# justinruggles/flake

Measured on AMD Instinct MI355X. Metric: Msamples/s encoded, 16-bit stereo 44.1k blocksize 4096 LPC-8, higher is better.
Workload: dtype int64/f64; 1 GPU; configs[1]: stereo 16-bit 44.1 kHz, blocksize 4096, LPC max order 8 (level-5 params, order method MAX, partition orders 0-5, stereo estimate), synthetic resonator PCM resident in HBM; frames_per_gpu=4096, batches=one resident batch, outputs=subframe info + packed Rice residual sections, parallelism=frame-sharded x1

## Files before the change

flake_amd/csrc/k1_autocorr.hip:

```cpp
#include "device_util.h"
#include "lpc_reg.h"

#ifdef FHIP_STAMPS
FHIP_DEFINE_STAMP_READER(fhip_debug_read_stamps_k1)
#define ACC_DECL(v_, n_) unsigned long long v_[n_] = {}
#define ACC_ADD(v_, i_, a_, b_) v_[i_] += (b_) - (a_)
#define ACC_PUT(slot_, val_)                                                           \
    do {                                                                               \
        if (blockIdx.x == 0 && (threadIdx.x & 63) == 0) g_fhip_stamps[slot_] = (long long)(val_); \
    } while (0)
#define STAMP_HWID() ACC_PUT(16 + (threadIdx.x >> 6), __builtin_amdgcn_s_getreg((31 << 11) | 4))
#else
#define ACC_DECL(v_, n_) do { } while (0)
#define ACC_ADD(v_, i_, a_, b_) do { } while (0)
#define ACC_PUT(slot_, val_) do { } while (0)
#define STAMP_HWID() do { } while (0)
#endif

namespace fhip {
namespace {

constexpr int AC_TILE = 128;
constexpr int AC_HALO = 32;
constexpr int AC_STRIDE = 170;
constexpr int AC_GMAX = 12;
constexpr int AC_PER_LANE = AC_TILE / WAVE;
constexpr int AC_CH = 8;
constexpr int AC_WAVES = 4;

__device__ __forceinline__ void wave_lds_fence()
{
    __builtin_amdgcn_fence(__ATOMIC_RELEASE, "wavefront");
    __builtin_amdgcn_wave_barrier();
    __builtin_amdgcn_fence(__ATOMIC_ACQUIRE, "wavefront");
}

__global__ __launch_bounds__(AC_WAVES * WAVE)
void k_autocorr(const int32_t *__restrict__ smp, double *__restrict__ autoc,
                int nsub, int n, int maxlag, int G, int nl2, double c, const int32_t *__restrict__ dev_sub)
{
    __shared__ double s_buf[AC_WAVES][AC_GMAX * AC_STRIDE];
    nsub = dev_count(dev_sub, nsub);

    const int lane = threadIdx.x & 63;
    const int wv = threadIdx.x >> 6;
    double *buf = s_buf[wv];
    const int s0 = (blockIdx.x * AC_WAVES + wv) * G;
    if (s0 >= nsub) return;
    const int half = n >> 1;
    const int ntiles = (n + AC_TILE - 1) / AC_TILE;

    const int32_t *rowp[AC_GMAX];
#pragma unroll
    for (int q = 0; q < AC_GMAX; q++) rowp[q] = smp + (size_t)min(s0 + q, nsub - 1) * n;
    int32_t cur[AC_GMAX][AC_PER_LANE];

    const int g = lane / nl2, j = lane - g * nl2;
    const int L0 = 2 * j, L1 = 2 * j + 1;
    const bool chain = (g < G) && (s0 + g < nsub) && (L0 <= maxlag);
    const double *rowa = buf + (chain ? g : 0) * AC_STRIDE + AC_HALO;
    const double *pb = rowa - (chain ? L0 : 0);
    double accE0 = 1.0, accO0 = 1.0, accE1 = 1.0, accO1 = 1.0;
    double b1 = 0.0;

    auto issue_loads = [&](int tb) {
#pragma unroll
        for (int q = 0; q < AC_GMAX; q++)
#pragma unroll
            for (int u = 0; u < AC_PER_LANE; u++)
                cur[q][u] = rowp[q][min(tb + u * WAVE + lane, n - 1)];
    };

    for (int idx = lane; idx < AC_GMAX * AC_HALO; idx += WAVE)
        buf[(idx >> 5) * AC_STRIDE + (idx & 31)] = 0.0;
    issue_loads(0);

    for (int t = 0; t < ntiles; t++) {
        const int tb = t * AC_TILE;
#pragma unroll
        for (int u = 0; u < AC_PER_LANE; u++) {
            const int p = tb + u * WAVE + lane;
            const int ii = (p < half) ? p : (n - 1 - p);
            const bool valid = (p < n) && (ii < half);
            const double tt = c - (double)ii;
            const double w = valid ? (1.0 - (tt * tt)) : 0.0;
#pragma unroll
            for (int q = 0; q < AC_GMAX; q++)
                buf[q * AC_STRIDE + AC_HALO + u * WAVE + lane] = (double)cur[q][u] * w;
        }
        issue_loads(tb + AC_TILE);
        wave_lds_fence();

        const int kend = min(AC_TILE, n - tb);
        if (t > 0 && kend == AC_TILE) {
            constexpr int NS = AC_TILE / AC_CH;
            double A[AC_CH], B[AC_CH], P[2 * AC_CH];
            double b1n;
            auto rd = [&](int st, double (&a)[AC_CH], double (&b)[AC_CH]) {
#pragma unroll
                for (int u = 0; u < AC_CH; u++) { a[u] = rowa[st * AC_CH + u]; b[u] = pb[st * AC_CH + u]; }
            };
            rd(0, A, B);
            {
                double pbv = b1;
#pragma unroll
                for (int u = 0; u < AC_CH; u++) { P[2 * u] = A[u] * B[u]; P[2 * u + 1] = A[u] * pbv; pbv = B[u]; }
                b1n = pbv;
            }
            rd(1, A, B);
#pragma unroll
            for (int cidx = 0; cidx < NS; cidx++) {
                double An[AC_CH], Bn[AC_CH], Pn[2 * AC_CH];
                if (cidx + 2 < NS) rd(cidx + 2, An, Bn);
                __builtin_amdgcn_sched_barrier(0);
                double pbv = b1n;
#pragma unroll
                for (int u = 0; u < AC_CH; u += 2) {
                    accE0 = accE0 + P[2 * u];
                    if (cidx + 1 < NS) Pn[2 * u] = A[u] * B[u];
                    accE1 = accE1 + P[2 * u + 1];
                    if (cidx + 1 < NS) Pn[2 * u + 1] = A[u] * pbv;
                    accO0 = accO0 + P[2 * u + 2];
                    if (cidx + 1 < NS) Pn[2 * u + 2] = A[u + 1] * B[u + 1];
                    accO1 = accO1 + P[2 * u + 3];
                    if (cidx + 1 < NS) Pn[2 * u + 3] = A[u + 1] * B[u];
                    pbv = B[u + 1];
                }
                __builtin_amdgcn_sched_barrier(0);
                if (cidx + 1 < NS) {
                    b1n = pbv;
#pragma unroll
                    for (int u = 0; u < 2 * AC_CH; u++) P[u] = Pn[u];
                }
                if (cidx + 2 < NS) {
#pragma unroll
                    for (int u = 0; u < AC_CH; u++) { A[u] = An[u]; B[u] = Bn[u]; }
                }
            }
            b1 = pb[AC_TILE - 1];
        } else {
            double accH0 = 1.0, accH1 = 1.0;
            for (int k = 0; k < kend; k++) {
                const int p = tb + k;
                const double a = rowa[k], b0 = pb[k];
                const double p0 = a * b0, p1 = a * b1;
                if (p <= maxlag) {
                    if (p >= L0) accH0 = accH0 + p0;
                    if (p >= L1) accH1 = accH1 + p1;
                    if (p == maxlag) {
                        if ((maxlag + 1) & 1) { accO0 = accH0; accO1 = accH1; }
                        else { accE0 = accH0; accE1 = accH1; }
                    }
                } else if (p & 1) {
                    accO0 = accO0 + p0;
                    accO1 = accO1 + p1;
                } else {
                    accE0 = accE0 + p0;
                    accE1 = accE1 + p1;
                }
                b1 = b0;
            }
        }
        wave_lds_fence();
        {
            double hv[(AC_GMAX * AC_HALO) / WAVE];
#pragma unroll
            for (int r = 0; r < (AC_GMAX * AC_HALO) / WAVE; r++) {
                const int idx = lane + r * WAVE;
                hv[r] = buf[(idx >> 5) * AC_STRIDE + AC_TILE + (idx & 31)];
            }
            wave_lds_fence();
#pragma unroll
            for (int r = 0; r < (AC_GMAX * AC_HALO) / WAVE; r++) {
                const int idx = lane + r * WAVE;
                buf[(idx >> 5) * AC_STRIDE + (idx & 31)] = hv[r];
            }
        }
    }
    if (chain) {
        double *dst = autoc + (size_t)(s0 + g) * FHIP_MAX_LAGS;
        dst[L0] = accE0 + accO0;
        if (L1 <= maxlag) dst[L1] = accE1 + accO1;
    }
}

__global__ __launch_bounds__(AC_WAVES * WAVE)
void k_autocorr_ragged(const int32_t *__restrict__ smp, double *__restrict__ autoc, int nsub, int nch, int row_n,
                       int maxlag, const int32_t *__restrict__ frame_n, const double *__restrict__ frame_c,
                       const int32_t *__restrict__ dev_sub)
{
    __shared__ double s_buf[AC_WAVES][AC_HALO + AC_TILE];
    const int lane = threadIdx.x & 63, wv = threadIdx.x >> 6;
    const int s = blockIdx.x * AC_WAVES + wv;
    nsub = dev_count(dev_sub, nsub);
    if (s >= nsub) return;
    double *buf = s_buf[wv];
    const int f = s / nch;
    const int n = __builtin_amdgcn_readfirstlane(frame_n[f]);
    double *dst = autoc + (size_t)s * FHIP_MAX_LAGS;
    if (n <= maxlag) {
        if (lane <= maxlag) dst[lane] = 2.0;
        return;
    }
    const double c = frame_c[f];
    const int32_t *row = smp + (size_t)s * row_n;
    const int half = n >> 1;
    const int lag = min(lane, maxlag);
    double acc1 = 1.0, acc2 = 1.0;
    if (lane < AC_HALO) buf[lane] = 0.0;
    for (int tb = 0; tb < n; tb += AC_TILE) {
#pragma unroll
        for (int u = 0; u < AC_PER_LANE; u++) {
            const int p = tb + u * WAVE + lane;
            const int ii = (p < half) ? p : (n - 1 - p);
            const bool valid = (p < n) && (ii < half);
            const double tt = c - (double)ii;
            const double w = valid ? (1.0 - (tt * tt)) : 0.0;
            buf[AC_HALO + u * WAVE + lane] = (double)row[min(p, n - 1)] * w;
        }
        wave_lds_fence();
        const int kend = min(AC_TILE, n - tb);
        for (int k = 0; k < kend; k++) {
            const int p = tb + k;
            const double prod = buf[AC_HALO + k] * buf[AC_HALO + k - lag];
            if (p <= maxlag) {
                if (p >= lag) acc1 = acc1 + prod;
            } else if ((p - maxlag) & 1) {
                acc1 = acc1 + prod;
            } else {
                acc2 = acc2 + prod;
            }
        }
        wave_lds_fence();
        const double hv = (lane < AC_HALO) ? buf[AC_TILE + lane] : 0.0;
        wave_lds_fence();
        if (lane < AC_HALO) buf[lane] = hv;
    }
    if (lane <= maxlag) dst[lane] = acc1 + acc2;
}

constexpr int PS_HALF = AC_TILE / 2;
constexpr int PS_HH = AC_HALO / 2;
constexpr int PS_ROW = PS_HH + PS_HALF;
constexpr int PS_STRIDE = 2 * PS_ROW + 10;
constexpr int PS_GMAX = 8;
constexpr int PS_CH = 8;

__global__ __launch_bounds__(AC_WAVES * WAVE)
void k_autocorr_ps(const int32_t *__restrict__ smp, double *__restrict__ autoc,
                   int nsub, int n, int maxlag, int G, int lps, int ge, double c,
                   const int32_t *__restrict__ dev_sub)
{
    __shared__ double s_buf[AC_WAVES][PS_GMAX * PS_STRIDE];
    nsub = dev_count(dev_sub, nsub);

    const int lane = threadIdx.x & 63;
    const int wv = threadIdx.x >> 6;
    double *buf = s_buf[wv];
    const int s0 = (blockIdx.x * AC_WAVES + wv) * G;
    if (s0 >= nsub) return;
    const int half = n >> 1;
    const int ntiles = (n + AC_TILE - 1) / AC_TILE;

    const int32_t *rowp[PS_GMAX];
#pragma unroll
    for (int q = 0; q < PS_GMAX; q++) rowp[q] = smp + (size_t)min(s0 + q, nsub - 1) * n;
    int32_t cur[PS_GMAX][AC_PER_LANE];

    const int g = lane / lps, ql = lane - g * lps;
    const int pi = ql & 1, grp = ql >> 1;
    const int l0 = (grp < ge) ? 6 * grp : 1 + 6 * (grp - ge);
    const bool chain = (g < G) && (s0 + g < nsub) && (l0 <= maxlag);
    const bool ok1 = l0 + 2 <= maxlag, ok2 = l0 + 4 <= maxlag;
    const int pib = pi ^ (l0 & 1);
    const int sft = (l0 + pib - pi) / 2;
    const double *rowA = buf + (chain ? g : 0) * PS_STRIDE + pi * PS_ROW + PS_HH;
    const double *rowB = buf + (chain ? g : 0) * PS_STRIDE + pib * PS_ROW + PS_HH - (chain ? sft : 0);
    const int pih = (maxlag + 1) & 1;
    double S0 = 1.0, S1 = 1.0, S2 = 1.0;
    double b1 = 0.0, b2 = 0.0;

    auto issue_loads = [&](int tb) {
#pragma unroll
        for (int q = 0; q < PS_GMAX; q++)
#pragma unroll
            for (int u = 0; u < AC_PER_LANE; u++)
                cur[q][u] = rowp[q][min(tb + u * WAVE + lane, n - 1)];
    };
    auto slot = [&](int q, int x) { return q * PS_STRIDE + (x & 1) * PS_ROW + PS_HH + (x >> 1); };

    for (int idx = lane; idx < PS_GMAX * 2 * PS_HH; idx += WAVE) {
        const int q = idx / (2 * PS_HH), r = idx - q * 2 * PS_HH;
        buf[q * PS_STRIDE + (r / PS_HH) * PS_ROW + (r % PS_HH)] = 0.0;
    }
    issue_loads(0);

    for (int t = 0; t < ntiles; t++) {
        const int tb = t * AC_TILE;
#pragma unroll
        for (int u = 0; u < AC_PER_LANE; u++) {
            const int x = u * WAVE + lane;
            const int p = tb + x;
            const int ii = (p < half) ? p : (n - 1 - p);
            const bool valid = (p < n) && (ii < half);
            const double tt = c - (double)ii;
            const double w = valid ? (1.0 - (tt * tt)) : 0.0;
#pragma unroll
            for (int q = 0; q < PS_GMAX; q++) buf[slot(q, x)] = (double)cur[q][u] * w;
        }
        issue_loads(tb + AC_TILE);
        wave_lds_fence();

        const int kend = min(AC_TILE, n - tb);
        if (t > 0 && kend == AC_TILE) {
            constexpr int NS = PS_HALF / PS_CH;
            double A[PS_CH], B[PS_CH];
#pragma unroll
            for (int u = 0; u < PS_CH; u++) { A[u] = rowA[u]; B[u] = rowB[u]; }
#pragma unroll
            for (int st = 0; st < NS; st++) {
                double An[PS_CH], Bn[PS_CH];
                if (st + 1 < NS) {
#pragma unroll
                    for (int u = 0; u < PS_CH; u++) {
                        An[u] = rowA[(st + 1) * PS_CH + u];
                        Bn[u] = rowB[(st + 1) * PS_CH + u];
                    }
                }
                __builtin_amdgcn_sched_barrier(0);
#pragma unroll
                for (int u = 0; u < PS_CH; u++) {
                    const double p0 = A[u] * B[u], p1 = A[u] * b1, p2 = A[u] * b2;
                    S0 = S0 + p0;
                    S1 = S1 + p1;
                    S2 = S2 + p2;
                    b2 = b1;
                    b1 = B[u];
                }
                __builtin_amdgcn_sched_barrier(0);
                if (st + 1 < NS) {
#pragma unroll
                    for (int u = 0; u < PS_CH; u++) { A[u] = An[u]; B[u] = Bn[u]; }
                }
            }
        } else {
            if (t == 0 && pi == pih) {
                const int hend = min(maxlag, kend - 1);
                for (int x = 0; x <= hend; x++) {
                    const double a = buf[slot(chain ? g : 0, x)];
                    if (x >= l0) {
                        const double p0 = a * buf[slot(chain ? g : 0, x - l0)];
                        S0 = S0 + p0;
                    }
                    if (ok1 && x >= l0 + 2) {
                        const double p1 = a * buf[slot(chain ? g : 0, x - l0 - 2)];
                        S1 = S1 + p1;
                    }
                    if (ok2 && x >= l0 + 4) {
                        const double p2 = a * buf[slot(chain ? g : 0, x - l0 - 4)];
                        S2 = S2 + p2;
                    }
                }
            }
            for (int st = 0; st < PS_HALF; st++) {
                const int x = 2 * st + pi;
                const int p = tb + x;
                if (x >= kend) break;
                const double a = rowA[st], b0 = rowB[st];
                if (p > maxlag) {
                    const double c1 = (x - l0 - 2 >= -AC_HALO) ? buf[slot(chain ? g : 0, x - l0 - 2 + AC_HALO) - PS_HH] : 0.0;
                    const double c2 = (x - l0 - 4 >= -AC_HALO) ? buf[slot(chain ? g : 0, x - l0 - 4 + AC_HALO) - PS_HH] : 0.0;
                    const double p0 = a * b0, p1 = a * c1, p2 = a * c2;
                    S0 = S0 + p0;
                    S1 = S1 + p1;
                    S2 = S2 + p2;
                }
                b2 = b1;
                b1 = b0;
            }
        }
        wave_lds_fence();
        {
            constexpr int NH = (PS_GMAX * 2 * PS_HH) / WAVE;
            double hv[NH];
#pragma unroll
            for (int r = 0; r < NH; r++) {
                const int idx = lane + r * WAVE;
                const int q = idx / (2 * PS_HH), rr = idx - q * 2 * PS_HH;
                hv[r] = buf[q * PS_STRIDE + (rr / PS_HH) * PS_ROW + PS_HALF + (rr % PS_HH)];
            }
            wave_lds_fence();
#pragma unroll
            for (int r = 0; r < NH; r++) {
                const int idx = lane + r * WAVE;
                const int q = idx / (2 * PS_HH), rr = idx - q * 2 * PS_HH;
                buf[q * PS_STRIDE + (rr / PS_HH) * PS_ROW + (rr % PS_HH)] = hv[r];
            }
        }
    }
    const double o0 = __shfl_xor(S0, 1, WAVE), o1 = __shfl_xor(S1, 1, WAVE), o2 = __shfl_xor(S2, 1, WAVE);
    if (chain && pi == 0) {
        double *dst = autoc + (size_t)(s0 + g) * FHIP_MAX_LAGS;
        dst[l0] = S0 + o0;
        if (ok1) dst[l0 + 2] = S1 + o1;
        if (ok2) dst[l0 + 4] = S2 + o2;
    }
}

template <int NCH, bool FUSED, int LPCMO>
constexpr wt_split wt_split_of() { return (NCH == 3 && !FUSED && LPCMO == 8) ? WT_SPLIT_O8 : WT_SPLIT_EVEN; }
constexpr int WT_ROW = PS_HH + PS_HALF + 2;
constexpr int WT_STRIDE = 2 * WT_ROW + 2;
static_assert(WT_ROW % 2 == 0 && WT_STRIDE % 4 == 2, "16-byte aligned arrays, odd slot stride");
constexpr int WT_BUF = WT_SUB * WT_STRIDE;
constexpr int WT_NBUF = 3;
#ifndef FHIP_WT_AHEAD
#define FHIP_WT_AHEAD 3
#endif
constexpr int WT_AHEAD = FHIP_WT_AHEAD;

template <int TL>
struct wt_geo {
    static_assert(TL == AC_TILE || TL == 2 * AC_TILE, "tile length");
    static constexpr int HALF = TL / 2;
    static constexpr int ROW = PS_HH + HALF + 2;
    static constexpr int STRIDE = 2 * ROW + 2;
    static constexpr int BUF = WT_SUB * STRIDE;
    static constexpr int NBUF = (TL == AC_TILE) ? WT_NBUF : 2;
    static constexpr int UNITS = TL / AC_TILE;
    static constexpr int AHEAD = (TL == AC_TILE) ? WT_AHEAD : 4;
    static constexpr int UT = AHEAD / UNITS;
    static_assert(ROW % 2 == 0 && STRIDE % 4 == 2, "16-byte aligned arrays, odd slot stride");
    static_assert(AHEAD % UNITS == 0 && (TL == AC_TILE || UT % NBUF == 0), "whole tiles per trip");
};
static_assert(wt_geo<AC_TILE>::ROW == WT_ROW && wt_geo<AC_TILE>::BUF == WT_BUF, "the 128 form's geometry");
constexpr int WTL_TILE = 2 * AC_TILE;

struct wt_groups { int l0[4]; int nch[4]; };

#ifdef FHIP_PROBE_NOB
constexpr bool wt_probe_nob = true;
#else
constexpr bool wt_probe_nob = false;
#endif
#ifdef FHIP_PROBE_NOPROD
constexpr bool wt_probe_noprod = true;
#else
constexpr bool wt_probe_noprod = false;
#endif
#ifdef FHIP_PROBE_NOWALK
constexpr bool wt_probe_nowalk = true;
#else
constexpr bool wt_probe_nowalk = false;
#endif
#ifdef FHIP_PROBE_NOHALO
constexpr bool wt_probe_nohalo = true;
#else
constexpr bool wt_probe_nohalo = false;
#endif
struct wt_lpc_args { int precision, omethod; int32_t *coefs, *shift, *opt_order, *fin; int32_t *tile_ctr; };
template <int MO>
__device__ __forceinline__ void lpc_reg_one(const double (&ac)[MO + 1], int s, int max_order, int precision,
                                            int omethod, int32_t *__restrict__ coefs,
                                            int32_t *__restrict__ shift, int32_t *__restrict__ opt_order,
                                            int32_t *__restrict__ fin);

template <int NCH, bool FUSED, int LPCMO, int TL>
__device__ __forceinline__
void wt_body(const int32_t *__restrict__ smp, double *__restrict__ autoc,
             int nsub, int n, int maxlag, wt_groups grp, double c,
             const int32_t *__restrict__ pcm, int32_t *__restrict__ smp_out,
             const fhip_subframe_info *__restrict__ info, wt_lpc_args lpc, int narrow_ok,
             const int32_t *__restrict__ dev_sub, const MultiBin &mb, wt_groups grp1, int lsplit)
{
    using GEO = wt_geo<TL>;
    constexpr int T_HALF = GEO::HALF, T_ROW = GEO::ROW, T_STRIDE = GEO::STRIDE, T_BUF = GEO::BUF;
    constexpr int T_NBUF = GEO::NBUF, T_UNITS = GEO::UNITS, T_AHEAD = GEO::AHEAD, T_UT = GEO::UT;
    constexpr bool LONG = TL != AC_TILE;
    extern __shared__ __attribute__((aligned(16))) double wt_lds[];
    double *acbuf = wt_lds + T_NBUF * T_BUF;

    const int lane = threadIdx.x & 63;
    const int wv = threadIdx.x >> 6;
    int blk = blockIdx.x;
    if (mb.nbins) {
        const int k = find_bin(mb, blk);
        blk -= mb.wg0[k];
        n = mb.n[k];
        c = mb.c[k];
        narrow_ok = mb.narrow[k];
        nsub = __builtin_amdgcn_readfirstlane(mb.cnt[mb.cnt_ix[k]]);
        const size_t u0 = (size_t)mb.unit0[k];
        smp += mb.smp_off[k];
        autoc += u0 * FHIP_MAX_LAGS;
        info += u0;
        lpc.coefs += u0 * FHIP_MAX_ORDER * FHIP_MAX_ORDER;
        lpc.shift += u0 * FHIP_MAX_ORDER;
        lpc.opt_order += u0;
        lpc.fin += u0 * FIN_STRIDE;
    } else {
        nsub = dev_count(dev_sub, nsub);
    }
    if (lsplit == 2) {
        if (blk & 1) grp = grp1;
        blk >>= 1;
    }
    const int sub0 = blk * WT_SUB;
    if (sub0 >= nsub) return;
    const int half = n >> 1;
    const int ntiles = n / TL;
    const int ntiles_pad = ((ntiles + T_UT - 1) / T_UT) * T_UT;
    STAMP_HWID();

    if (wv >= 4) {
        auto produce = [&](auto nrows_c, int q0, auto allnar_c) {
            constexpr int NR = decltype(nrows_c)::value;
            constexpr bool ALLNAR = decltype(allnar_c)::value;
            constexpr int NL = FUSED ? (NR + 1) / 2 : NR;
            auto uni64 = [](unsigned long long v) {
                return ((unsigned long long)(unsigned)__builtin_amdgcn_readfirstlane((int)(v >> 32)) << 32) |
                       (unsigned)__builtin_amdgcn_readfirstlane((int)v);
            };
            unsigned long long rowb[NL], outb[NR];
            int mode[NL], w0s[NL], w1s[NL];
            int nar[NL];
#pragma unroll
            for (int r = 0; r < NL; r++) {
                if (FUSED) {
                    const int sub = min(sub0 + q0 + 2 * r, nsub - 2);
                    rowb[r] = uni64((unsigned long long)(pcm + (size_t)sub * n));
                    outb[2 * r] = uni64((unsigned long long)(smp_out + (size_t)sub * n));
                    outb[2 * r + 1] = uni64((unsigned long long)(smp_out + (size_t)(sub + 1) * n));
                    mode[r] = __builtin_amdgcn_readfirstlane(info[sub].ch_mode);
                    w0s[r] = __builtin_amdgcn_readfirstlane(info[sub].wasted);
                    w1s[r] = __builtin_amdgcn_readfirstlane(info[sub + 1].wasted);
                } else {
                    const int sub = min(sub0 + q0 + r, nsub - 1);
                    rowb[r] = uni64((unsigned long long)(smp + (size_t)sub * n));
                    nar[r] = narrow_ok ? (__builtin_amdgcn_readfirstlane(info[sub].reserved) & 0xFF) : 0;
                }
            }
            typedef typename std::conditional<FUSED, int4, int2>::type ld_t;
            ld_t pre[T_AHEAD][NL];
            auto issue_loads = [&](ld_t (&dst)[NL], int tb, bool pinned = false) {
                const int p = min(tb + 2 * lane, n - 2);
#pragma unroll
                for (int r = 0; r < NL; r++) {
                    const int idx = FUSED ? 2 * p : ((ALLNAR || nar[r]) ? (p >> 1) : p);
                    typedef const int32_t __attribute__((address_space(1))) *g_i32;
                    typedef int ldv_t __attribute__((ext_vector_type(FUSED ? 4 : 2)));
                    typedef const ldv_t __attribute__((address_space(1))) *g_ld;
                    if constexpr (ALLNAR) {
                        dst[r].x = *((g_i32)rowb[r] + idx);
                    } else {
                        const ldv_t v = *(g_ld)((g_i32)rowb[r] + idx);
                        __builtin_memcpy(&dst[r], &v, sizeof(ld_t));
                    }
                    if (pinned) __builtin_amdgcn_sched_barrier(0);
                }
            };
#pragma unroll
            for (int a = 0; a < T_AHEAD; a++) issue_loads(pre[a], a * AC_TILE, true);
            if constexpr (!LONG) {
                for (int idx = lane; idx < NR * 2 * PS_HH; idx += WAVE) {
                    const int r = idx / (2 * PS_HH), k = idx - r * 2 * PS_HH;
                    wt_lds[(q0 + r) * T_STRIDE + (k / PS_HH) * T_ROW + (k % PS_HH)] = 0.0;
                }
            }
            double hl0[LONG ? NR : 1], hl1[LONG ? NR : 1];
#pragma unroll
            for (int r = 0; r < (LONG ? NR : 1); r++) { hl0[r] = 0.0; hl1[r] = 0.0; }
            auto weight = [&](int p) {
                const int ii = (p < half) ? p : (n - 1 - p);
                const bool valid = (p < n) && (ii < half);
                const double tt = c - (double)ii;
                return valid ? (1.0 - (tt * tt)) : 0.0;
            };
            int bi = 0;
            ACC_DECL(pacc, 3);
            for (int t0 = 0; t0 < ntiles_pad; t0 += T_UT) {
#pragma unroll
                for (int a = 0; a < T_UT; a++) {
                    const int bnx = (bi == T_NBUF - 1) ? 0 : bi + 1;
                    const bool tail = lane >= PS_HALF - PS_HH;
                    if (LONG && tail && !wt_probe_nohalo && !wt_probe_noprod) {
                        double *bh = wt_lds + bi * T_BUF + q0 * T_STRIDE + lane - (PS_HALF - PS_HH);
#pragma unroll
                        for (int r = 0; r < NR; r++) {
                            bh[r * T_STRIDE] = hl0[LONG ? r : 0];
                            bh[r * T_STRIDE + T_ROW] = hl1[LONG ? r : 0];
                        }
                    }
#pragma unroll
                    for (int h = 0; h < T_UNITS; h++) {
                        TICK(tp0);
                        const int ai = a * T_UNITS + h;
                        const int tb = (t0 + a) * TL + h * AC_TILE;
                        double *bw = wt_lds + bi * T_BUF + q0 * T_STRIDE + PS_HH + h * PS_HALF + lane;
                        double *bn = wt_lds + bnx * T_BUF + q0 * T_STRIDE + PS_HH + lane - PS_HALF;
                        const double w0 = weight(tb + 2 * lane), w1 = weight(tb + 2 * lane + 1);
                        const int pst = min(tb + 2 * lane, n - 2);
                        double hv0[NR], hv1[NR];
#pragma unroll
                        for (int r = 0; r < (wt_probe_noprod ? 0 : NR); r++) {
                            int32_t x0, x1;
                            if (FUSED) {
                                const int4 v = *reinterpret_cast<const int4 *>(&pre[ai][r / 2]);
                                const int md = mode[r / 2];
                                const int32_t s0 = (int32_t)((uint32_t)v.x - (uint32_t)v.y);
                                const int32_t s1 = (int32_t)((uint32_t)v.z - (uint32_t)v.w);
                                if ((r & 1) == 0) {
                                    const int32_t m0 = (int32_t)((uint32_t)v.x + (uint32_t)v.y) >> 1;
                                    const int32_t m1 = (int32_t)((uint32_t)v.z + (uint32_t)v.w) >> 1;
                                    x0 = (md == FHIP_CH_MID_SIDE) ? m0 : (md == FHIP_CH_RIGHT_SIDE) ? s0 : v.x;
                                    x1 = (md == FHIP_CH_MID_SIDE) ? m1 : (md == FHIP_CH_RIGHT_SIDE) ? s1 : v.z;
                                    x0 >>= w0s[r / 2]; x1 >>= w0s[r / 2];
                                } else {
                                    x0 = (md == FHIP_CH_MID_SIDE || md == FHIP_CH_LEFT_SIDE) ? s0 : v.y;
                                    x1 = (md == FHIP_CH_MID_SIDE || md == FHIP_CH_LEFT_SIDE) ? s1 : v.w;
                                    x0 >>= w1s[r / 2]; x1 >>= w1s[r / 2];
                                }
                                *reinterpret_cast<int2 *>(reinterpret_cast<int32_t *>(outb[r]) + pst) = make_int2(x0, x1);
                            } else {
                                const int2 v = *reinterpret_cast<const int2 *>(&pre[ai][r]);
                                const bool nr = ALLNAR || nar[FUSED ? 0 : r] != 0;
                                x0 = nr ? (int32_t)(int16_t)v.x : v.x;
                                x1 = nr ? (v.x >> 16) : v.y;
                            }
                            const double v0 = (double)x0 * w0;
                            const double v1 = (double)x1 * w1;
#ifdef FHIP_PROBE_NOLDSW
                            if (r == 0) { hv0[0] = 0; hv1[0] = 0; }
                            hv0[0] += v0; hv1[0] += v1;
                            if (r == NR - 1) { bw[0] = hv0[0]; bw[T_ROW] = hv1[0]; }
#else
                            bw[r * T_STRIDE] = v0;
                            bw[r * T_STRIDE + T_ROW] = v1;
                            hv0[r] = v0; hv1[r] = v1;
#endif
                        }
                        if constexpr (LONG) {
                            if (h == T_UNITS - 1) {
#pragma unroll
                                for (int r = 0; r < NR; r++) { hl0[r] = hv0[r]; hl1[r] = hv1[r]; }
                            }
                        } else if (tail && !wt_probe_nohalo && !wt_probe_noprod) {
#pragma unroll
                            for (int r = 0; r < NR; r++) {
                                bn[r * T_STRIDE] = hv0[r];
                                bn[r * T_STRIDE + T_ROW] = hv1[r];
                            }
                        }
                        TICK(tp1);
                        issue_loads(pre[ai], tb + T_AHEAD * AC_TILE);
                        TICK(tp2);
                        ACC_ADD(pacc, 0, tp0, tp1); ACC_ADD(pacc, 1, tp1, tp2);
                        if (h < T_UNITS - 1) {
                            __builtin_amdgcn_sched_barrier(0);
                        }
                    }
                    TICK(tp2);
                    __syncthreads();
                    TICK(tp3);
                    ACC_ADD(pacc, 2, tp2, tp3);
                    __builtin_amdgcn_sched_barrier(0);
                    bi = bnx;
                }
            }
            ACC_PUT(wv - 4, pacc[0]); ACC_PUT(wv, pacc[1]); ACC_PUT(wv + 4, pacc[2]);
            if (wv == 4) { ACC_PUT(44, pacc[0]); ACC_PUT(45, pacc[1]); ACC_PUT(46, pacc[2]); }
        };
        constexpr wt_split SP = wt_split_of<NCH, FUSED, LPCMO>();
        static_assert(wt_split_valid(SP), "producer row split");
        const int q0w = (wv == 4) ? 0 : (wv == 5) ? wt_split_first(SP, 1) : (wv == 6) ? wt_split_first(SP, 2)
                                                                                      : wt_split_first(SP, 3);
        const int nrw = (wv == 4) ? SP.rows[0] : (wv == 5) ? SP.rows[1] : (wv == 6) ? SP.rows[2] : SP.rows[3];
        bool alln = !FUSED && narrow_ok != 0;
        if (alln) {
            const int wide = (info[min(sub0 + q0w + min(lane, nrw - 1), nsub - 1)].reserved & 0xFF) == 0;
            alln = __ballot(wide) == 0;
        }
        auto produce_rows = [&](auto kc) {
            constexpr int K = decltype(kc)::value;
            if constexpr (wt_split_first_with(SP, K)) {
                if (nrw == SP.rows[K]) {
                    if (alln) produce(std::integral_constant<int, SP.rows[K]>{}, q0w, std::true_type{});
                    else produce(std::integral_constant<int, SP.rows[K]>{}, q0w, std::false_type{});
                }
            }
        };
        produce_rows(std::integral_constant<int, 0>{});
        produce_rows(std::integral_constant<int, 1>{});
        produce_rows(std::integral_constant<int, 2>{});
        produce_rows(std::integral_constant<int, 3>{});
        if (LPCMO > 0) __syncthreads();
        return;
    }

    const int pi = lane >> 5, sl = lane & 31;
    const int l0 = wv == 0 ? grp.l0[0] : wv == 1 ? grp.l0[1] : wv == 2 ? grp.l0[2] : grp.l0[3];
    const int nch = wv == 0 ? grp.nch[0] : wv == 1 ? grp.nch[1] : wv == 2 ? grp.nch[2] : grp.nch[3];
    const bool live = (sub0 + sl < nsub) && nch > 0;
    const int pib = pi ^ (l0 & 1);
    const int sft = (l0 + pib - pi) / 2;
    const int offA = sl * T_STRIDE + pi * T_ROW + PS_HH;
    const int offB = sl * T_STRIDE + pib * T_ROW + PS_HH - sft;
    const int pih = (maxlag + 1) & 1;
    auto slotc = [&](int x) { return sl * T_STRIDE + (x & 1) * T_ROW + PS_HH + (x >> 1); };
    double S[NCH], cy[NCH];
#pragma unroll
    for (int j = 0; j < NCH; j++) { S[j] = 1.0; cy[j] = 0.0; }

    auto walk_tile = [&](const double *rowA_, const double *rowB_, auto first, auto same, auto histc, auto kc,
                         auto &hist) {
        constexpr bool FIRST = decltype(first)::value;
        constexpr bool SAME = decltype(same)::value;
        constexpr int HD = decltype(histc)::value;
        constexpr int K = decltype(kc)::value;
        constexpr bool NOB = SAME || HD > 0 || wt_probe_nob;
        constexpr int NS = T_HALF / PS_CH;
        constexpr int DEPTH = (K <= 3) ? 2 : 1;
        constexpr int NSET = DEPTH + 1;
        typedef const volatile double __attribute__((address_space(3))) lds_cvd;
        typedef double dbl2 __attribute__((ext_vector_type(2)));
        typedef const volatile dbl2 __attribute__((address_space(3))) lds_cvd2;
        lds_cvd2 *rowA = (lds_cvd2 *)rowA_;
        lds_cvd *rowB = (lds_cvd *)rowB_;
        double A[NSET][PS_CH], B[NSET][PS_CH];
        int maxlag_v = maxlag;
        if constexpr (FIRST) asm volatile("" : "+v"(maxlag_v));
        auto fetch = [&](int set, int stage) {
#pragma unroll
            for (int u = 0; u < PS_CH; u += 2) {
                const dbl2 v = rowA[(stage * PS_CH + u) / 2];
                A[set][u] = v.x; A[set][u + 1] = v.y;
            }
            if (!NOB) {
#pragma unroll
                for (int u = 0; u < PS_CH; u++) B[set][u] = rowB[stage * PS_CH + u];
            }
        };
        constexpr int PER_STAGE = PS_CH / 2 + (NOB ? 0 : PS_CH);
        auto stage = [&](int st, int set, bool ahead, int newer, bool headz) __attribute__((always_inline)) {
            if (ahead) fetch((set + DEPTH) % NSET, st + DEPTH);
            {
                constexpr int w1 = PER_STAGE > 15 ? 15 : PER_STAGE;
                constexpr int w2 = 2 * PER_STAGE > 15 ? 15 : 2 * PER_STAGE;
                constexpr int enc1 = (3 << 14) | (w1 << 8) | (7 << 4) | 0xF;
                constexpr int enc2 = (3 << 14) | (w2 << 8) | (7 << 4) | 0xF;
                constexpr int enc0 = (3 << 14) | (0 << 8) | (7 << 4) | 0xF;
                if (newer == 2) __builtin_amdgcn_s_waitcnt(enc2);
                else if (newer == 1) __builtin_amdgcn_s_waitcnt(enc1);
                else __builtin_amdgcn_s_waitcnt(enc0);
            }
            __builtin_amdgcn_sched_barrier(0);
#pragma unroll
            for (int u = 0; u < PS_CH; u++) {
                const double x = (SAME || wt_probe_nob) ? A[set][u] : (HD > 0) ? hist[HD > 0 ? HD - 1 : 0]
                                                                                : B[set][u];
                double a = A[set][u];
                if (FIRST && headz && 2 * (st * PS_CH + u) <= FHIP_MAX_ORDER)
                    a = (2 * (st * PS_CH + u) + pi > maxlag_v) ? a : 0.0;
                double pr[K];
                pr[0] = a * x;
#pragma unroll
                for (int j = 1; j < K; j++) pr[j] = a * cy[j];
#pragma unroll
                for (int j = 0; j < K; j++) S[j] = S[j] + pr[j];
#pragma unroll
                for (int j = K - 1; j >= 2; j--) cy[j] = cy[j - 1];
                if constexpr (K > 1) cy[1] = x;
                if constexpr (HD > 0) {
#pragma unroll
                    for (int k = HD - 1; k >= 1; k--) hist[k] = hist[k - 1];
                    hist[0] = A[set][u];
                }
            }
            __builtin_amdgcn_sched_barrier(0);
        };
        auto newer_of = [](int st) { return (st + DEPTH < NS ? 1 : 0) + ((DEPTH == 2 && st + 1 < NS) ? 1 : 0); };
#pragma unroll
        for (int k = 0; k < DEPTH; k++) fetch(k, k);
        if constexpr (!LONG) {
#pragma unroll
            for (int st = 0; st < NS; st++) stage(st, st % NSET, st + DEPTH < NS, newer_of(st), true);
        } else {
            constexpr int HEADST = FIRST ? ((FHIP_MAX_ORDER / 2 + PS_CH) / PS_CH + NSET - 1) / NSET * NSET : 0;
            constexpr int STEADY = (NS - DEPTH) / NSET * NSET;
            static_assert(HEADST <= STEADY && (!FIRST || HEADST * PS_CH * 2 > FHIP_MAX_ORDER), "head inside the peeled stages");
#pragma unroll
            for (int st = 0; st < HEADST; st++) stage(st, st % NSET, true, DEPTH, true);
#pragma unroll 1
            for (int st0 = HEADST; st0 < STEADY; st0 += NSET) {
#pragma unroll
                for (int s = 0; s < NSET; s++) stage(st0 + s, s, true, DEPTH, false);
            }
#pragma unroll
            for (int st = STEADY; st < NS; st++) stage(st, st % NSET, st + DEPTH < NS, newer_of(st), false);
        }
    };

    auto walk_all = [&](auto same, auto histc, auto kc) {
        constexpr int HD = decltype(histc)::value;
        double hist[HD > 0 ? HD : 1];
#pragma unroll
        for (int k = 0; k < (HD > 0 ? HD : 1); k++) hist[k] = 0.0;
        int bi = 0;
        ACC_DECL(cacc, 4);
        for (int t = 0; t < ntiles_pad; t++) {
            TICK(tc0);
            __syncthreads();
            TICK(tc1);
            ACC_ADD(cacc, 0, tc0, tc1);
            if (t == 0) ACC_ADD(cacc, 3, tc0, tc1);
            if (t >= ntiles || wt_probe_nowalk || nch <= 0) continue;
            const double *buf = wt_lds + bi * T_BUF;
            if (t == 0 && pi == pih) {
#ifndef FHIP_HEAD_LOOP
                if constexpr (LPCMO > 0 && NCH >= 3) {
                    double hd[LPCMO + 1], he[LPCMO + 1];
#pragma unroll
                    for (int x = 0; x <= LPCMO; x++) { hd[x] = buf[slotc(x)]; he[x] = buf[slotc(x - l0)]; }
#pragma unroll
                    for (int x = 0; x <= LPCMO; x++) {
                        const double a = (x <= maxlag) ? hd[x] : 0.0;
#pragma unroll
                        for (int j = 0; j < NCH; j++) {
                            if (x - 2 * j >= 0) {
                                const double pr = a * he[x - 2 * j];
                                S[j] = S[j] + pr;
                            }
                        }
                    }
                } else
#endif
                for (int x = 0; x <= maxlag; x++) {
                    const double a = buf[slotc(x)];
#pragma unroll
                    for (int j = 0; j < NCH; j++) {
                        const int lag = l0 + 2 * j;
                        if (j < nch && x >= lag) {
                            const double pr = a * buf[slotc(x - lag)];
                            S[j] = S[j] + pr;
                        }
                    }
                }
            }
            if (t == 0) walk_tile(buf + offA, buf + offB, std::true_type{}, same, histc, kc, hist);
            else walk_tile(buf + offA, buf + offB, std::false_type{}, same, histc, kc, hist);
            bi = (bi == T_NBUF - 1) ? 0 : bi + 1;
            TICK(tc2);
            if (t == 0) ACC_ADD(cacc, 2, tc1, tc2);
            else ACC_ADD(cacc, 1, tc1, tc2);
        }
        ACC_PUT(48 + wv, cacc[1]); ACC_PUT(52 + wv, cacc[2]); ACC_PUT(56 + wv, cacc[0]); ACC_PUT(60 + wv, cacc[3]);
        if (wv == 0) { ACC_PUT(40, cacc[0]); ACC_PUT(41, cacc[1]); ACC_PUT(42, cacc[2]); }
    };

    using KF = std::integral_constant<int, NCH>;
    using KL = std::integral_constant<int, (NCH > 1) ? NCH - 1 : 1>;
    using H0 = std::integral_constant<int, 0>;
    using HN = std::integral_constant<int, NCH>;
    if (l0 == 0) {
        walk_all(std::true_type{}, H0{}, KF{});
    } else if (l0 == 2 * NCH) {
        if (nch == NCH) walk_all(std::false_type{}, HN{}, KF{});
        else walk_all(std::false_type{}, HN{}, KL{});
    } else if (nch == NCH) {
        walk_all(std::false_type{}, H0{}, KF{});
    } else {
        walk_all(std::false_type{}, H0{}, KL{});
    }
#pragma unroll
    for (int j = 0; j < NCH; j++) {
        const double o = __shfl_xor(S[j], 32, WAVE);
        if (live && pi == 0 && j < nch) {
            const double v = S[j] + o;
            autoc[(size_t)(sub0 + sl) * FHIP_MAX_LAGS + l0 + 2 * j] = v;
            if (LPCMO > 0) acbuf[sl * FHIP_MAX_LAGS + l0 + 2 * j] = v;
        }
    }
    if constexpr (LPCMO > 0) {
        bool tail_here = true;
        if (lsplit == 2) {
            asm volatile("s_waitcnt vmcnt(0)" ::: "memory");
            __syncthreads();
            int last = 0;
            if (threadIdx.x == 0) {
                __builtin_amdgcn_fence(__ATOMIC_RELEASE, "agent");
                asm volatile("s_waitcnt vmcnt(0)" ::: "memory");
                const int ticket = __hip_atomic_fetch_add(&lpc.tile_ctr[blk], 1, __ATOMIC_RELAXED, __HIP_MEMORY_SCOPE_AGENT);
                last = ticket & 1;
                if (last) {
                    __builtin_amdgcn_fence(__ATOMIC_ACQUIRE, "agent");
                    asm volatile("s_waitcnt vmcnt(0)" ::: "memory");
                }
            }
            tail_here = wv == 0 && __builtin_amdgcn_readfirstlane(last) != 0;
        } else {
            __syncthreads();
        }
        if (tail_here && wv == 0 && lane < WT_SUB && sub0 + lane < nsub) {
            double ac[LPCMO + 1];
            if (lsplit == 2) {
                const double *row = autoc + (size_t)(sub0 + lane) * FHIP_MAX_LAGS;
#pragma unroll
                for (int i = 0; i <= LPCMO; i++) ac[i] = (i <= maxlag) ? row[i] : 0.0;
            } else {
#pragma unroll
                for (int i = 0; i <= LPCMO; i++) ac[i] = (i <= maxlag) ? acbuf[lane * FHIP_MAX_LAGS + i] : 0.0;
            }
            lpc_reg_one<LPCMO>(ac, sub0 + lane, maxlag, lpc.precision, lpc.omethod, lpc.coefs, lpc.shift,
                               lpc.opt_order, lpc.fin);
        }
    }
}

#define WT_KERNEL_ARGS                                                                              \
    const int32_t *__restrict__ smp, double *__restrict__ autoc, int nsub, int n, int maxlag,       \
    wt_groups grp, double c, const int32_t *__restrict__ pcm, int32_t *__restrict__ smp_out,        \
    const fhip_subframe_info *__restrict__ info, wt_lpc_args lpc, int narrow_ok,                    \
    const int32_t *__restrict__ dev_sub, MultiBin mb, wt_groups grp1, int lsplit
#define WT_KERNEL_PASS smp, autoc, nsub, n, maxlag, grp, c, pcm, smp_out, info, lpc, narrow_ok, dev_sub, mb, grp1, lsplit

template <int NCH, bool FUSED, int LPCMO>
__global__ __launch_bounds__(8 * WAVE)
void k_autocorr_wt(WT_KERNEL_ARGS)
{
    wt_body<NCH, FUSED, LPCMO, AC_TILE>(WT_KERNEL_PASS);
}

template <int NCH, bool FUSED, int LPCMO>
__global__ __launch_bounds__(8 * WAVE)
void k_autocorr_wtl(WT_KERNEL_ARGS)
{
    wt_body<NCH, FUSED, LPCMO, WTL_TILE>(WT_KERNEL_PASS);
}
#undef WT_KERNEL_ARGS
#undef WT_KERNEL_PASS

}

namespace {
struct ac_choice { int kernel; int G, nl2, Gp, lps, ge, ne, no, split; };
ac_choice pick_autocorr(int nsub, int n, int max_order)
{
    ac_choice ch{};
    const int simds = 1024;
    ch.nl2 = (max_order + 2) / 2;
    ch.G = WAVE / ch.nl2;
    if (ch.G > AC_GMAX) ch.G = AC_GMAX;
    if (ch.G < 1) ch.G = 1;
    const long waves_cur = (nsub + ch.G - 1) / ch.G;
    ch.ne = max_order / 2 + 1; ch.no = (max_order + 1) / 2;
    ch.ge = (ch.ne + 2) / 3;
    const int go = (ch.no + 2) / 3;
    ch.lps = 2 * (ch.ge + go);
    ch.Gp = WAVE / ch.lps;
    if (ch.Gp > PS_GMAX) ch.Gp = PS_GMAX;
    const double t_cur = (double)((waves_cur + 2 * simds - 1) / (2 * simds)) *
                         (n * (waves_cur > simds ? 41.0 : 33.0) + 1000.0);
    const double t_ps = (ch.Gp >= 1) ? (double)(((nsub + ch.Gp - 1) / ch.Gp + simds - 1) / simds) * (0.5 * n * 39.0 + 1000.0) : 1e30;
    double t_wt = 1e30;
    ch.split = 1;
    if ((n % AC_TILE) == 0) {
        const int e0 = (ch.ne + 1) / 2;
        const double per_step = (4.8 * e0 > 23.0) ? 4.8 * e0 : 23.0;
        const int tiles = (nsub + WT_SUB - 1) / WT_SUB;
        t_wt = (double)((tiles + 255) / 256) * (0.5 * n * per_step + 8000.0);
        static const bool no_split = getenv("FHIP_NO_LAG_SPLIT") != nullptr;
        if (!no_split && 2 * tiles <= 256 && max_order >= 2) {
            ch.split = 2;
            const int m = (ch.ne + 3) / 4;
            const double ps2 = (4.8 * m > 14.0) ? 4.8 * m : 14.0;
            t_wt = 0.5 * n * ps2 + 8000.0;
        }
    }
    const double k2 = (max_order <= 12) ? 9000.0 : 0.0;
    ch.kernel = (t_wt <= t_ps + k2 && t_wt <= t_cur + k2) ? 2 : (t_ps < t_cur) ? 1 : 0;
    if (const char *force = getenv("FHIP_AC_KERNEL")) {
        if (force[0] == 'c') ch.kernel = 0;
        if (force[0] == 'p' && ch.Gp >= 1) ch.kernel = 1;
        if (force[0] == 'w' && (n % AC_TILE) == 0) ch.kernel = 2;
    }
    return ch;
}

bool wt_long_tile(const int *n, int count)
{
    const char *force = getenv("FHIP_WT_TILE");
    if (force && atoi(force) == AC_TILE) return false;
    for (int k = 0; k < count; k++) if (n[k] < WTL_TILE || (n[k] % WTL_TILE) != 0) return false;
    return true;
}
constexpr size_t wt_lds_bytes(bool long_tile)
{
    return sizeof(double) * (long_tile ? (size_t)wt_geo<WTL_TILE>::NBUF * wt_geo<WTL_TILE>::BUF
                                       : (size_t)WT_NBUF * WT_BUF);
}
static_assert(wt_lds_bytes(true) + sizeof(double) * WT_SUB * FHIP_MAX_LAGS <= 160 * 1024, "one workgroup's LDS");
}

}

extern "C" FHIP_API int fhip_autocorr_tile(int nsub, int n, int max_order)
{
    if (nsub < 1 || n < 1 || max_order < 1 || max_order > FHIP_MAX_ORDER) return 0;
    if (fhip::pick_autocorr(nsub, n, max_order).kernel != 2) return 0;
    return fhip::wt_long_tile(&n, 1) ? fhip::WTL_TILE : fhip::AC_TILE;
}

namespace fhip {

bool autocorr_is_wave_typed(int nsub, int n, int max_order)
{
    return pick_autocorr(nsub, n, max_order).kernel == 2;
}


bool autocorr_does_lpc(int nsub, int n, int max_order, bool have_tile_counters)
{
    static const bool off = getenv("FHIP_NO_LPC_TAIL") != nullptr;
    static const bool split_tail = getenv("FHIP_SPLIT_TAIL") != nullptr;
    if (off || max_order > 12) return false;
    const ac_choice ch = pick_autocorr(nsub, n, max_order);
    return ch.kernel == 2 && (ch.split == 1 || (have_tile_counters && split_tail));
}

bool autocorr_fuses_prepare(const fhip_params &p, int nsub, int n)
{
    static const bool on = getenv("FHIP_FUSE") != nullptr;
    if (!on || p.channels != 2 || (n & 3) != 0 || n > 4096 || (nsub & 1)) return false;
    return pick_autocorr(nsub, n, p.max_prediction_order).kernel == 2;
}

bool autocorr_bins_supported(int max_order, const int *n, int nbins)
{
    static const bool off = getenv("FHIP_NO_MULTIBIN") != nullptr;
    if (off || nbins < 1 || nbins > 8 || max_order < 1 || max_order > FHIP_MAX_ORDER) return false;
    for (int k = 0; k < nbins; k++) if (n[k] < AC_TILE || (n[k] % AC_TILE) != 0 || n[k] <= max_order) return false;
    return true;
}

hipError_t launch_autocorr_bins(hipStream_t st, const MultiBin &mb, const int32_t *smp, int max_order,
                                double *autoc, const fhip_subframe_info *info,
                                const autocorr_lpc_out *lpc_out)
{
    if (!autocorr_bins_supported(max_order, mb.n, mb.nbins)) return hipErrorInvalidValue;
    const int ne = max_order / 2 + 1, no = (max_order + 1) / 2;
    const int e0 = (ne + 1) / 2, e1 = ne - e0, o0 = (no + 1) / 2, o1 = no - o0;
    wt_groups gr;
    gr.l0[0] = 0;          gr.nch[0] = e0;
    gr.l0[1] = 2 * e0;     gr.nch[1] = e1;
    gr.l0[2] = 1;          gr.nch[2] = o0;
    gr.l0[3] = 1 + 2 * o0; gr.nch[3] = o1;
    const int nch = e0;
    const int blocks = mb.wg0[mb.nbins];
    if (blocks == 0) return hipSuccess;
    wt_lpc_args la{};
    int lpcmo = 0;
    if (lpc_out) {
        if (max_order > 12) return hipErrorInvalidValue;
        la.precision = lpc_out->precision; la.omethod = lpc_out->omethod;
        la.coefs = lpc_out->coefs; la.shift = lpc_out->shift; la.opt_order = lpc_out->opt_order;
        la.fin = lpc_out->fin;
        lpcmo = (max_order <= 8) ? 8 : 12;
    }
    const bool long_tile = wt_long_tile(mb.n, mb.nbins);
    const size_t lds = wt_lds_bytes(long_tile) + (lpcmo ? sizeof(double) * (size_t)WT_SUB * FHIP_MAX_LAGS : 0);
    bool any_narrow = false;
    for (int k = 0; k < mb.nbins; k++) any_narrow = any_narrow || mb.narrow[k];
#define LAUNCH_WTB(N_, L_)                                                                 \
    do {                                                                                     \
        auto kern = long_tile ? &k_autocorr_wtl<N_, false, L_> : &k_autocorr_wt<N_, false, L_>; \
        hipError_t er = hipFuncSetAttribute(reinterpret_cast<const void *>(kern),            \
                                            hipFuncAttributeMaxDynamicSharedMemorySize, (int)lds); \
        if (er != hipSuccess) return er;                                                     \
        note_launch("k_autocorr_wt<%d,false,%d> split=1%s%s", N_, L_, L_ ? " tail" : "", any_narrow ? " narrow" : ""); \
        hipLaunchKernelGGL(kern, dim3(blocks), dim3(8 * WAVE), lds, st, smp,                 \
                           autoc, 0, 0, max_order, gr, 0.0, (const int32_t *)nullptr, (int32_t *)nullptr, info, la, 0, \
                           (const int32_t *)nullptr, mb, wt_groups{}, 1);                    \
    } while (0)
    if (lpcmo == 8) {
        switch (nch) {
        case 1: LAUNCH_WTB(1, 8); break;
        case 2: LAUNCH_WTB(2, 8); break;
        case 3: LAUNCH_WTB(3, 8); break;
        default: return hipErrorInvalidValue;
        }
    } else if (lpcmo == 12) {
        switch (nch) {
        case 3: LAUNCH_WTB(3, 12); break;
        case 4: LAUNCH_WTB(4, 12); break;
        default: return hipErrorInvalidValue;
        }
    } else {
        switch (nch) {
        case 1: LAUNCH_WTB(1, 0); break;
        case 2: LAUNCH_WTB(2, 0); break;
        case 3: LAUNCH_WTB(3, 0); break;
        case 4: LAUNCH_WTB(4, 0); break;
        case 5: LAUNCH_WTB(5, 0); break;
        case 6: LAUNCH_WTB(6, 0); break;
        case 7: LAUNCH_WTB(7, 0); break;
        case 8: LAUNCH_WTB(8, 0); break;
        case 9: LAUNCH_WTB(9, 0); break;
        default: return hipErrorInvalidValue;
        }
    }
#undef LAUNCH_WTB
    return hipGetLastError();
}

hipError_t launch_autocorr_ragged(hipStream_t st, const int32_t *smp, int nsub, int nch, const RaggedFrames &rf,
                                  int max_order, double *autoc)
{
    if (nsub == 0) return hipSuccess;
    if (!rf.frame_n || !rf.frame_c || max_order < 1 || max_order > FHIP_MAX_ORDER) return hipErrorInvalidValue;
    note_launch("k_autocorr ragged");
    hipLaunchKernelGGL(k_autocorr_ragged, dim3((nsub + AC_WAVES - 1) / AC_WAVES), dim3(AC_WAVES * WAVE), 0, st, smp,
                       autoc, nsub, nch, rf.row_n, max_order, rf.frame_n, rf.frame_c, rf.dev_sub);
    return hipGetLastError();
}

hipError_t launch_autocorr(hipStream_t st, const int32_t *smp, int nsub, int n,
                           int max_order, double *autoc, const int32_t *pcm_fused,
                           int32_t *smp_out, const fhip_subframe_info *info,
                           const autocorr_lpc_out *lpc_out, bool narrow_ok, const int32_t *dev_sub,
                           int nsub_hint)
{
    if (nsub == 0) return hipSuccess;
    const double c = (2.0 / (n - 1.0)) - 1.0;
    const ac_choice ch = pick_autocorr(nsub_hint > 0 ? nsub_hint : nsub, n, max_order);
    const int ne = ch.ne, no = ch.no, Gp = ch.Gp, lps = ch.lps, ge = ch.ge, nl2 = ch.nl2;
    int G = ch.G;
    const bool use_wt = ch.kernel == 2, use_ps = ch.kernel == 1;
    if ((pcm_fused || lpc_out || narrow_ok) && !use_wt) return hipErrorInvalidValue;
    if (narrow_ok && (!info || pcm_fused)) return hipErrorInvalidValue;
    const int e0 = (ne + 1) / 2, e1 = ne - e0, o0 = (no + 1) / 2, o1 = no - o0;
    if (use_wt) {
        wt_groups gr, gr1{};
        const int split = (pcm_fused || (lpc_out && !lpc_out->tile_ctr)) ? 1 : ch.split;
        int nch;
        if (split == 2) {
            auto spread = [](wt_groups &g, int first, int count) {
                int l = first;
                for (int w = 0; w < 4; w++) {
                    const int k = count / 4 + (w < count % 4 ? 1 : 0);
                    g.l0[w] = l; g.nch[w] = k;
                    l += 2 * k;
                }
            };
            spread(gr, 0, ne);
            spread(gr1, 1, no);
            nch = (ne + 3) / 4;
        } else {
            gr.l0[0] = 0;          gr.nch[0] = e0;
            gr.l0[1] = 2 * e0;     gr.nch[1] = e1;
            gr.l0[2] = 1;          gr.nch[2] = o0;
            gr.l0[3] = 1 + 2 * o0; gr.nch[3] = o1;
            nch = e0;
        }
        const int blocks = split * ((nsub + WT_SUB - 1) / WT_SUB);
        const bool long_tile = !pcm_fused && wt_long_tile(&n, 1);
        const size_t lds = wt_lds_bytes(long_tile);
        wt_lpc_args la{};
        int lpcmo = 0;
        if (lpc_out) {
            if (max_order > 12 || pcm_fused) return hipErrorInvalidValue;
            la.precision = lpc_out->precision; la.omethod = lpc_out->omethod;
            la.coefs = lpc_out->coefs; la.shift = lpc_out->shift; la.opt_order = lpc_out->opt_order;
            la.fin = lpc_out->fin; la.tile_ctr = lpc_out->tile_ctr;
            lpcmo = (max_order <= 8) ? 8 : 12;
        }
        const size_t lds_all = lds + (lpcmo ? sizeof(double) * (size_t)WT_SUB * FHIP_MAX_LAGS : 0);
#define LAUNCH_WT3(N_, F_, L_)                                                               \
    do {                                                                                     \
        auto kern = (long_tile && !F_) ? &k_autocorr_wtl<N_, false, L_> : &k_autocorr_wt<N_, F_, L_>; \
        hipError_t er = hipFuncSetAttribute(reinterpret_cast<const void *>(kern),            \
                                            hipFuncAttributeMaxDynamicSharedMemorySize, (int)lds_all); \
        if (er != hipSuccess) return er;                                                     \
        note_launch("k_autocorr_wt<%d,%s,%d> split=%d%s%s%s", N_, tf(F_), L_, split, L_ ? " tail" : "", \
                    F_ ? " fused" : "", narrow_ok ? " narrow" : "");                         \
        hipLaunchKernelGGL(kern, dim3(blocks), dim3(8 * WAVE), lds_all, st, smp,             \
                           autoc, nsub, n, max_order, gr, c, pcm_fused, smp_out, info, la, narrow_ok ? 1 : 0, dev_sub, MultiBin{}, gr1, split); \
    } while (0)
#define LAUNCH_WT(N_)                                                                        \
    case N_:                                                                                 \
        if (pcm_fused) LAUNCH_WT3(N_, true, 0); else LAUNCH_WT3(N_, false, 0);               \
        break;
        if (lpcmo == 8) {
            switch (nch) {
            case 1: LAUNCH_WT3(1, false, 8); break;
            case 2: LAUNCH_WT3(2, false, 8); break;
            case 3: LAUNCH_WT3(3, false, 8); break;
            default: return hipErrorInvalidValue;
            }
            return hipGetLastError();
        }
        if (lpcmo == 12) {
            switch (nch) {
            case 2: LAUNCH_WT3(2, false, 12); break;
            case 3: LAUNCH_WT3(3, false, 12); break;
            case 4: LAUNCH_WT3(4, false, 12); break;
            default: return hipErrorInvalidValue;
            }
            return hipGetLastError();
        }
        switch (nch) {
            LAUNCH_WT(1) LAUNCH_WT(2) LAUNCH_WT(3) LAUNCH_WT(4) LAUNCH_WT(5)
            LAUNCH_WT(6) LAUNCH_WT(7) LAUNCH_WT(8) LAUNCH_WT(9)
        default: return hipErrorInvalidValue;
        }
#undef LAUNCH_WT
#undef LAUNCH_WT3
        return hipGetLastError();
    }
    if (use_ps) {
        const int per_block = Gp * AC_WAVES;
        const int blocks = (nsub + per_block - 1) / per_block;
        note_launch("k_autocorr_ps");
        hipLaunchKernelGGL(k_autocorr_ps, dim3(blocks), dim3(AC_WAVES * WAVE), 0, st, smp, autoc,
                           nsub, n, max_order, Gp, lps, ge, c, dev_sub);
        return hipGetLastError();
    }
    while (G > 1 && (nsub + G * AC_WAVES - 1) / (G * AC_WAVES) < 256) G--;
    if (const char *dbg = getenv("FHIP_AC_G")) { int v = atoi(dbg); if (v >= 1 && v <= AC_GMAX && v * nl2 <= WAVE) G = v; }
    const int per_block = G * AC_WAVES;
    const int blocks = (nsub + per_block - 1) / per_block;
    note_launch("k_autocorr");
    hipLaunchKernelGGL(k_autocorr, dim3(blocks), dim3(AC_WAVES * WAVE), 0, st, smp, autoc,
                       nsub, n, max_order, G, nl2, c, dev_sub);
    return hipGetLastError();
}

}
```

Before: 254,400 Msamples/s.

## Peel padded tail tiles, use byte offsets for loads, split LDS prefetch into early/late

The weighting loop is split so that full tiles run through a branch-free window weight, and only the final padded trip keeps the bounds checks. Global load addressing is rewritten to use precomputed unsigned byte offsets instead of per-row index arithmetic. In the autocorrelation stage pipeline, the A operands are kept as double2 vectors, and part of the next-stage LDS prefetch is deferred until the registers holding the tail data are free. The waitcnt thresholds are adjusted to match the new issue order. The aim is to cut ALU and addressing overhead and lower VGPR pressure, at the cost of more complex wait-count bookkeeping that could be gotten wrong.

```diff
diff --git a/flake_amd/csrc/k1_autocorr.hip b/flake_amd/csrc/k1_autocorr.hip
--- a/flake_amd/csrc/k1_autocorr.hip
+++ b/flake_amd/csrc/k1_autocorr.hip
@@ -544,16 +544,19 @@
             ld_t pre[T_AHEAD][NL];
             auto issue_loads = [&](ld_t (&dst)[NL], int tb, bool pinned = false) {
                 const int p = min(tb + 2 * lane, n - 2);
+                const unsigned off_w = (unsigned)p * (FUSED ? 8u : 4u);
+                const unsigned off_n = (unsigned)(p >> 1) * 4u;
 #pragma unroll
                 for (int r = 0; r < NL; r++) {
-                    const int idx = FUSED ? 2 * p : ((ALLNAR || nar[r]) ? (p >> 1) : p);
+                    const unsigned off = FUSED ? off_w : ((ALLNAR || nar[r]) ? off_n : off_w);
+                    typedef const char __attribute__((address_space(1))) *g_byte;
                     typedef const int32_t __attribute__((address_space(1))) *g_i32;
                     typedef int ldv_t __attribute__((ext_vector_type(FUSED ? 4 : 2)));
                     typedef const ldv_t __attribute__((address_space(1))) *g_ld;
                     if constexpr (ALLNAR) {
-                        dst[r].x = *((g_i32)rowb[r] + idx);
+                        dst[r].x = *(g_i32)((g_byte)rowb[r] + off);
                     } else {
-                        const ldv_t v = *(g_ld)((g_i32)rowb[r] + idx);
+                        const ldv_t v = *(g_ld)((g_byte)rowb[r] + off);
                         __builtin_memcpy(&dst[r], &v, sizeof(ld_t));
                     }
                     if (pinned) __builtin_amdgcn_sched_barrier(0);
@@ -570,15 +573,20 @@
             double hl0[LONG ? NR : 1], hl1[LONG ? NR : 1];
 #pragma unroll
             for (int r = 0; r < (LONG ? NR : 1); r++) { hl0[r] = 0.0; hl1[r] = 0.0; }
-            auto weight = [&](int p) {
-                const int ii = (p < half) ? p : (n - 1 - p);
-                const bool valid = (p < n) && (ii < half);
-                const double tt = c - (double)ii;
-                return valid ? (1.0 - (tt * tt)) : 0.0;
+            auto weight = [&](int p, auto pad_c) {
+                if constexpr (decltype(pad_c)::value) {
+                    const int ii = (p < half) ? p : (n - 1 - p);
+                    const bool valid = (p < n) && (ii < half);
+                    const double tt = c - (double)ii;
+                    return valid ? (1.0 - (tt * tt)) : 0.0;
+                } else {
+                    const double tt = c - (double)min(p, n - 1 - p);
+                    return 1.0 - (tt * tt);
+                }
             };
             int bi = 0;
             ACC_DECL(pacc, 3);
-            for (int t0 = 0; t0 < ntiles_pad; t0 += T_UT) {
+            auto trip = [&](int t0, auto pad_c) {
 #pragma unroll
                 for (int a = 0; a < T_UT; a++) {
                     const int bnx = (bi == T_NBUF - 1) ? 0 : bi + 1;
@@ -598,7 +606,7 @@
                         const int tb = (t0 + a) * TL + h * AC_TILE;
                         double *bw = wt_lds + bi * T_BUF + q0 * T_STRIDE + PS_HH + h * PS_HALF + lane;
                         double *bn = wt_lds + bnx * T_BUF + q0 * T_STRIDE + PS_HH + lane - PS_HALF;
-                        const double w0 = weight(tb + 2 * lane), w1 = weight(tb + 2 * lane + 1);
+                        const double w0 = weight(tb + 2 * lane, pad_c), w1 = weight(tb + 2 * lane + 1, pad_c);
                         const int pst = min(tb + 2 * lane, n - 2);
                         double hv0[NR], hv1[NR];
 #pragma unroll
@@ -666,7 +674,10 @@
                     __builtin_amdgcn_sched_barrier(0);
                     bi = bnx;
                 }
-            }
+            };
+            int t0 = 0;
+            for (; t0 + T_UT <= ntiles; t0 += T_UT) trip(t0, std::false_type{});
+            if (t0 < ntiles_pad) trip(t0, std::true_type{});
             ACC_PUT(wv - 4, pacc[0]); ACC_PUT(wv, pacc[1]); ACC_PUT(wv + 4, pacc[2]);
             if (wv == 4) { ACC_PUT(44, pacc[0]); ACC_PUT(45, pacc[1]); ACC_PUT(46, pacc[2]); }
         };
@@ -726,26 +737,39 @@
         typedef const volatile dbl2 __attribute__((address_space(3))) lds_cvd2;
         lds_cvd2 *rowA = (lds_cvd2 *)rowA_;
         lds_cvd *rowB = (lds_cvd *)rowB_;
-        double A[NSET][PS_CH], B[NSET][PS_CH];
+        dbl2 A[NSET][PS_CH / 2];
+        double B[NSET][PS_CH];
         int maxlag_v = maxlag;
         if constexpr (FIRST) asm volatile("" : "+v"(maxlag_v));
+        constexpr int TAILN = (HD > 0 ? HD : 0) + K - 1;
+        constexpr bool LATE_OK = LONG && DEPTH == 2 && TAILN >= 1 && TAILN <= PS_CH - 2;
+        constexpr int LATEQ = (NOB && LATE_OK) ? (TAILN + 1) / 2 : 0;
+        constexpr int LATEB = (!NOB && LATE_OK) ? TAILN : 0;
+        constexpr int EARLYQ = PS_CH / 2 - LATEQ, EARLYB = PS_CH - LATEB;
+        auto fetch_a = [&](int set, int stage, int q0, int q1) {
+#pragma unroll
+            for (int q = q0; q < q1; q++) A[set][q] = rowA[(stage * PS_CH) / 2 + q];
+        };
+        auto fetch_b = [&](int set, int stage, int u0, int u1) {
+            if (!NOB) {
+#pragma unroll
+                for (int u = u0; u < u1; u++) B[set][u] = rowB[stage * PS_CH + u];
+            }
+        };
         auto fetch = [&](int set, int stage) {
-#pragma unroll
-            for (int u = 0; u < PS_CH; u += 2) {
-                const dbl2 v = rowA[(stage * PS_CH + u) / 2];
-                A[set][u] = v.x; A[set][u + 1] = v.y;
-            }
-            if (!NOB) {
-#pragma unroll
-                for (int u = 0; u < PS_CH; u++) B[set][u] = rowB[stage * PS_CH + u];
-            }
+            fetch_a(set, stage, 0, PS_CH / 2);
+            fetch_b(set, stage, 0, PS_CH);
         };
         constexpr int PER_STAGE = PS_CH / 2 + (NOB ? 0 : PS_CH);
         auto stage = [&](int st, int set, bool ahead, int newer, bool headz) __attribute__((always_inline)) {
-            if (ahead) fetch((set + DEPTH) % NSET, st + DEPTH);
+            if (ahead) {
+                fetch_a((set + DEPTH) % NSET, st + DEPTH, 0, EARLYQ);
+                fetch_b((set + DEPTH) % NSET, st + DEPTH, 0, EARLYB);
+            }
             {
                 constexpr int w1 = PER_STAGE > 15 ? 15 : PER_STAGE;
-                constexpr int w2 = 2 * PER_STAGE > 15 ? 15 : 2 * PER_STAGE;
+                constexpr int w2r = 2 * PER_STAGE - LATEQ - LATEB;
+                constexpr int w2 = w2r > 15 ? 15 : w2r;
                 constexpr int enc1 = (3 << 14) | (w1 << 8) | (7 << 4) | 0xF;
                 constexpr int enc2 = (3 << 14) | (w2 << 8) | (7 << 4) | 0xF;
                 constexpr int enc0 = (3 << 14) | (0 << 8) | (7 << 4) | 0xF;
@@ -756,9 +780,15 @@
             __builtin_amdgcn_sched_barrier(0);
 #pragma unroll
             for (int u = 0; u < PS_CH; u++) {
-                const double x = (SAME || wt_probe_nob) ? A[set][u] : (HD > 0) ? hist[HD > 0 ? HD - 1 : 0]
-                                                                                : B[set][u];
-                double a = A[set][u];
+                if (LATEQ + LATEB > 0 && ahead && u == TAILN) {
+                    __builtin_amdgcn_sched_barrier(0);
+                    fetch_a((set + DEPTH) % NSET, st + DEPTH, EARLYQ, PS_CH / 2);
+                    fetch_b((set + DEPTH) % NSET, st + DEPTH, EARLYB, PS_CH);
+                    __builtin_amdgcn_sched_barrier(0);
+                }
+                const double au = (u & 1) ? A[set][u / 2].y : A[set][u / 2].x;
+                const double x = (SAME || wt_probe_nob) ? au : (HD > 0) ? hist[HD > 0 ? HD - 1 : 0] : B[set][u];
+                double a = au;
                 if (FIRST && headz && 2 * (st * PS_CH + u) <= FHIP_MAX_ORDER)
                     a = (2 * (st * PS_CH + u) + pi > maxlag_v) ? a : 0.0;
                 double pr[K];
@@ -773,7 +803,7 @@
                 if constexpr (HD > 0) {
 #pragma unroll
                     for (int k = HD - 1; k >= 1; k--) hist[k] = hist[k - 1];
-                    hist[0] = A[set][u];
+                    hist[0] = au;
                 }
             }
             __builtin_amdgcn_sched_barrier(0);
```

Result: no change. 256,900 Msamples/s, median of 6 (+1.0%).
